# erwincoumans/tiny-differentiable-simulator

Hardware: AMD Instinct MI355X
Metric: env-steps/sec (higher is better)
Workload: dtype f64

## Files before the change

tiny-differentiable-simulator_amd/csrc/tds_oct.hip:

```cpp
#include <hip/hip_runtime.h>
#include <stdlib.h>

#include "tds_device_model.h"
#include "tds_kernels.h"
#include "tds_lanes.h"
#include "tds_step_shared.h"

#ifdef TDS_OCT_PROF
#ifndef TDS_OCT_PROF_WG
#define TDS_OCT_PROF_WG 3
#endif
__device__ unsigned long long tds_oct_prof_buf[32];
__device__ unsigned long long tds_oct_prof_clk[64];
__device__ unsigned long long tds_oct_prof_wg[3 * 2048];
__device__ int tds_oct_prof_iter = 500;
#define OCT_STAMP(k, pin)                                                                       \
  do {                                                                                          \
    unsigned long long t_;                                                                      \
    auto p_ = (pin);        \
    asm volatile("s_memtime %0\n\ts_waitcnt lgkmcnt(0)" : "=s"(t_), "+v"(p_)::"memory");        \
    if (prof_on) prof_t[k] = t_;                                                                \
  } while (0)
#else
#define OCT_STAMP(k, pin) do { } while (0)
#endif

#ifdef TDS_OCT_MARKS
#define OCT_MARK(name) asm volatile("; OCTMARK " name ::: "memory")
#else
#define OCT_MARK(name) do { } while (0)
#endif

namespace {

#define OCT_SYNC()                                             \
  do {                                                         \
    __builtin_amdgcn_fence(__ATOMIC_ACQ_REL, "wavefront");     \
    __builtin_amdgcn_wave_barrier();                           \
  } while (0)

template <int CTRL>
__device__ __forceinline__ double oct_dpp(double v) {
  const int l = __double2loint(v), h = __double2hiint(v);
  const int lo = __builtin_amdgcn_update_dpp(0, l, CTRL, 0xF, 0xF, true);
  const int hi = __builtin_amdgcn_update_dpp(0, h, CTRL, 0xF, 0xF, true);
  return __hiloint2double(hi, lo);
}
template <int CTRL>
__device__ __forceinline__ float oct_dpp(float v) {
  return __int_as_float(__builtin_amdgcn_update_dpp(0, __float_as_int(v), CTRL, 0xF, 0xF, true));
}
template <typename T>
__device__ __forceinline__ T pair_other(T v) { return oct_dpp<0xB1>(v); }
template <int K, typename T>
__device__ __forceinline__ T pair_bcast(T v) { return oct_dpp<(K == 0 ? 0xA0 : 0xF5)>(v); }
template <typename T>
__device__ __forceinline__ T oct_sum(T v) {
  asm volatile("" : "+v"(v));
  v += oct_dpp<0xB1>(v);
  v += oct_dpp<0x4E>(v);
  v += oct_dpp<0x141>(v);
  return v;
}
template <int K>
__device__ __forceinline__ double oct_bcast(double v) {
  const double t = __builtin_amdgcn_update_dpp(0.0, v, 0x150 + K, 0xF, 0x3, false);
  return __builtin_amdgcn_update_dpp(t, v, 0x150 + 8 + K, 0xF, 0xC, false);
}
template <int K>
__device__ __forceinline__ float oct_bcast(float v) {
  const int b = __float_as_int(v);
  const int t = __builtin_amdgcn_update_dpp(0, b, 0x150 + K, 0xF, 0x3, false);
  return __int_as_float(__builtin_amdgcn_update_dpp(t, b, 0x150 + 8 + K, 0xF, 0xC, false));
}

struct OctOff {
  int lcw, legf, swl, qdp, fac, win, xs, cp, stride;
};
struct OctLds {
  static constexpr int LCW = 6;
  static constexpr int ZW = 14;
  static constexpr int Z_B = 10, Z_A = 11, Z_G = 12, Z_HL = 13;
  static constexpr int NCP = 17;
};
__host__ __device__ inline OctOff oct_layout(int in_dim) {
  OctOff o;
  int at = in_dim + 4;
  at = (at + 1) & ~1;
  o.lcw = at;  at += 8 * OctLds::LCW;
  o.legf = at; at += 4 * 3;
  o.swl = at;  at += 8 * 6;
  o.qdp = at;  at += 8;
  o.fac = at;  at += 28;
  o.win = at;  at += 2 * 8 * OctLds::ZW;
  o.xs = at;   at += 3 * OctLds::NCP + 1;
  o.cp = at;   at += 5 * OctLds::NCP + 1;
  at = (at + 1) & ~1;
  while ((((at * 2) & 63) % 8) != 0 || ((at * 2) & 63) == 0 || ((at * 2) & 63) == 32) at += 2;
  o.stride = at;
  return o;
}

struct OctKernArgs {
  const void *mdl, *x_in;
  void *y_out;
  const void *actions;
  void *x_feedback, *obs_out;
  TdsStepCtl ctl;
  int n_envs;
  OctOff O;
};
using TB = TdsOctTab;

#ifdef TDS_OCT_NT
#define OCT_ST(v, p) __builtin_nontemporal_store((v), (p))
#else
#define OCT_ST(v, p) (*(p) = (v))
#endif
#define OCT_BAR()                                                                        \
  do {                                                                                   \
    if constexpr (W2) asm volatile("s_waitcnt lgkmcnt(0)\n\ts_barrier" ::: "memory");    \
    else OCT_SYNC();                                                                     \
  } while (0)

template <typename T, typename TR, bool LOOP, int BUILD>
__device__ __forceinline__ void oct_body(const DevModel<T> *__restrict__ mdl_arg, const TR *x_in, TR *__restrict__ y_out,
                                         const TR *__restrict__ actions, TR *x_feedback ,
                                         TR *__restrict__ obs_out, const TdsStepCtl &ctl_arg, int n_envs, const OctOff &O) {
  extern __shared__ __align__(16) unsigned char tds_oct_smem[];
  T *const sm = reinterpret_cast<T *>(tds_oct_smem);
#ifdef TDS_OCT_PROF
  if (threadIdx.x == 0 && blockIdx.x < 2048) {
    unsigned long long c_;
    asm volatile("s_memrealtime %0\n\ts_waitcnt lgkmcnt(0)" : "=s"(c_)::"memory");
    tds_oct_prof_wg[3 * blockIdx.x] = c_;
  }
#endif
  constexpr bool W2 = BUILD >= 2;
  constexpr int nq = 14, nd = 14, adim = 8, in_dim = nq + nd + adim + 3, w_obs = nq + nd + 2;
  constexpr int NT = W2 ? 128 : 64;
  T *const CT = sm + 8 * O.stride;
  {
    const int t = threadIdx.x;
// ... 66 lines not shown
    asm volatile("s_memtime %0\n\ts_memrealtime %1\n\ts_waitcnt lgkmcnt(0)" : "=s"(c0_), "=s"(c1_)::"memory");
    tds_oct_prof_clk[2 * it] = c0_;
    tds_oct_prof_clk[2 * it + 1] = c1_;
  }
#endif
  const int lane = tid & 7;
  const int grp = (tid & 63) >> 3;
  const int env = blockIdx.x * 8 + grp;
  const bool valid = env < n_envs;
  T *const E = sm + grp * O.stride;
  T *const xr = E;
  const int leg = lane >> 1, pos = lane & 1;
  const int dq = 6 + lane;
  const T *const CL = CT + lane * TB::LSTR;
  typename TdsCtlRef<LOOP>::type ctl = TdsCtlRef<LOOP>::get(ctl_arg, ka_seg + __builtin_offsetof(OctKernArgs, ctl));
  const T dt = CT[TB::SC + TB::DT];
  const int pgs_iters = (int)CT[TB::SC + TB::PGS_ITERATIONS];
  const bool last = it == nsteps - 1;
  OCT_STAMP(0, tid);

  T q, qd, tau;
  T Sl[6], R[9], p[3], sw[6], v[6], a0[6];
  T R5[9], P[3], A4[3], A5[3], pA3[3], pA4[3], pA5[3], v5[6], a5[6];
  T Lc[6], l10, id0, id1, sq0, sq1, my_id, my_sq, Ls[15], ids[6], sq_ids[6], qd_new, qdr_new[6];
  T Cb, Cr[6], It[10];
  T u = T(0), urm = T(0);
  T u_init = T(0), urm_init = T(0);
  int na = 0, NA = 0;

  auto root_frame = [&](T sx, T cx, T sy, T cy, T sz, T cz) {
    R5[0] = cy * cz;                 R5[1] = -cy * sz;                R5[2] = sy;
    R5[3] = sx * sy * cz + cx * sz;  R5[4] = cx * cz - sx * sy * sz;  R5[5] = -sx * cy;
    R5[6] = sx * sz - cx * sy * cz;  R5[7] = cx * sy * sz + sx * cz;  R5[8] = cx * cy;
    P[0] = xr[0] + CT[TB::SC + TB::BASE_T];
    P[1] = xr[1] + CT[TB::SC + TB::BASE_T + 1];
    P[2] = xr[2] + CT[TB::SC + TB::BASE_T + 2];
    A4[0] = T(0); A4[1] = cx; A4[2] = sx;
    A5[0] = sy; A5[1] = -sx * cy; A5[2] = cx * cy;
    pA3[0] = T(0); pA3[1] = P[2]; pA3[2] = -P[1];
    cross3(P, A4, pA4);
    cross3(P, A5, pA5);
  };
  auto times_inertia = [&](const T *I, const T *s, T *F) {
    T t3[3];
    sym3_mulv(I, s, F);
    cross3(I + 6, s + 3, t3);
    F[0] += t3[0];
    F[1] += t3[1];
    F[2] += t3[2];
    cross3(I + 6, s, t3);
    F[3] = I[9] * s[3] - t3[0];
    F[4] = I[9] * s[4] - t3[1];
    F[5] = I[9] * s[5] - t3[2];
  };
  auto dot6 = [&](const T *a, const T *b) -> T { return dot3(a, b) + dot3(a + 3, b + 3); };

  auto main_kin = [&]() {
    OCT_MARK("main_top");
    q = xr[dq];
    qd = xr[nq + dq];
    tau = T(0);
    {
      const int act_i = act_slot;
      if (act_i >= 0) {
        const int var = nq + nd + adim;
        const T kp = xr[var], kd = xr[var + 1], max_force = xr[var + 2];
        const T act_lim = CT[TB::SC + TB::ACTION_LIMIT];
        T a = xr[nq + nd + act_i];
        a = a < act_lim ? a : act_lim;
        a = a > -act_lim ? a : -act_lim;
        const T q_des = CL[TB::IPOSE] + a;
        T f = kp * (q_des - q) + kd * (T(0) - qd);
        f = f > -max_force ? f : -max_force;
        f = f < max_force ? f : max_force;
        tau = f;
      }
      tau -= CL[TB::STIFF] * q + CL[TB::DAMP] * qd;
      asm volatile("" : "+v"(tau));
    }
    OCT_MARK("main_jcalc");
#pragma unroll
    for (int k = 0; k < 6; ++k) Sl[k] = CL[TB::S + k];
    T Rp[9], tp[3];
    {
      T sn, cs;
      tds_sincos(q * CL[TB::ROTF], &sn, &cs);
      const T c1 = T(1) - cs;
      const T nx = CL[TB::NAX], ny = CL[TB::NAX + 1], nz = CL[TB::NAX + 2];
      T RJ[9];
      RJ[0] = cs + c1 * CL[TB::NN + 0];
      RJ[1] = c1 * CL[TB::NN + 1] - sn * nz;
      RJ[2] = c1 * CL[TB::NN + 2] + sn * ny;
      RJ[3] = c1 * CL[TB::NN + 1] + sn * nz;
      RJ[4] = cs + c1 * CL[TB::NN + 3];
      RJ[5] = c1 * CL[TB::NN + 4] - sn * nx;
      RJ[6] = c1 * CL[TB::NN + 2] - sn * ny;
      RJ[7] = c1 * CL[TB::NN + 4] + sn * nx;
      RJ[8] = cs + c1 * CL[TB::NN + 5];
      const T tJ[3] = {Sl[3] * q, Sl[4] * q, Sl[5] * q};
      if (CT[TB::SC + TB::XT_IDENT] != T(0)) {
#pragma unroll
        for (int k = 0; k < 9; ++k) Rp[k] = RJ[k];
#pragma unroll
        for (int k = 0; k < 3; ++k) tp[k] = CL[TB::XT + 9 + k] + tJ[k];
      } else {
        T RT[9], r[3];
#pragma unroll
        for (int k = 0; k < 9; ++k) RT[k] = CL[TB::XT + k];
        mat3_mul(RT, RJ, Rp);
        mat3_mulv(RT, tJ, r);
#pragma unroll
        for (int k = 0; k < 3; ++k) tp[k] = CL[TB::XT + 9 + k] + r[k];
      }
    }
    OCT_MARK("main_rootsincos");
    {
      T rs, rc;
      tds_sincos(xr[3 + (lane < 3 ? lane : 0)], &rs, &rc);
      const T sx = oct_bcast<0>(rs), cx = oct_bcast<0>(rc);
      const T sy = oct_bcast<1>(rs), cy = oct_bcast<1>(rc);
      const T sz = oct_bcast<2>(rs), cz = oct_bcast<2>(rc);
      if constexpr (W2) {
        if (lane < 3) {
          T *const sc = E + O.win + 8 * OctLds::ZW + 96;
          sc[2 * lane] = rs;
          sc[2 * lane + 1] = rc;
        }
      }
      root_frame(sx, cx, sy, cy, sz, cz);
    }
    OCT_MARK("main_rootvel");
    {
      const T d0 = xr[nq + 0], d1 = xr[nq + 1], d2 = xr[nq + 2], d3 = xr[nq + 3], d4 = xr[nq + 4], d5 = xr[nq + 5];
      const T U[3] = {d0, d1, d2};
      const T J3[3] = {d3, T(0), T(0)}, J4[3] = {A4[0] * d4, A4[1] * d4, A4[2] * d4}, J5[3] = {A5[0] * d5, A5[1] * d5, A5[2] * d5};
      const T W4[3] = {J3[0] + J4[0], J3[1] + J4[1], J3[2] + J4[2]};
      const T W5[3] = {W4[0] + J5[0], W4[1] + J5[1], W4[2] + J5[2]};
      T pJ3[3], pJ4[3], pJ5[3];
      cross3(P, J3, pJ3);
      cross3(P, J4, pJ4);
      cross3(P, J5, pJ5);
      const T pW4[3] = {pJ3[0] + pJ4[0], pJ3[1] + pJ4[1], pJ3[2] + pJ4[2]};
      const T pW5[3] = {pW4[0] + pJ5[0], pW4[1] + pJ5[1], pW4[2] + pJ5[2]};
      const T V3[3] = {U[0] + pJ3[0], U[1] + pJ3[1], U[2] + pJ3[2]};
      const T V4[3] = {U[0] + pW4[0], U[1] + pW4[1], U[2] + pW4[2]};
      const T V5[3] = {U[0] + pW5[0], U[1] + pW5[1], U[2] + pW5[2]};
      T a45[3], a55[3], t1[3], t2[3], l3[3], l4[3], l5[3];
      cross3(J3, J4, a45);
      cross3(W4, J5, a55);
      cross3(J3, pJ3, t1);
      cross3(V3, J3, t2);
      l3[0] = t1[0] + t2[0]; l3[1] = t1[1] + t2[1]; l3[2] = t1[2] + t2[2];
      cross3(W4, pJ4, t1);
      cross3(V4, J4, t2);
      l4[0] = t1[0] + t2[0]; l4[1] = t1[1] + t2[1]; l4[2] = t1[2] + t2[2];
      cross3(W5, pJ5, t1);
      cross3(V5, J5, t2);
      l5[0] = t1[0] + t2[0]; l5[1] = t1[1] + t2[1]; l5[2] = t1[2] + t2[2];
#pragma unroll
      for (int k = 0; k < 3; ++k) {
        v5[k] = W5[k];
        v5[3 + k] = V5[k];
        a5[k] = a45[k] + a55[k];
        a5[3 + k] = (l3[k] + l4[k] + l5[k]) - CT[TB::SC + TB::GRAV + k];
      }
    }
    OCT_MARK("main_legs");
    {
      const bool take = pos == 1;
      T Rq[9], pq[3];
#pragma unroll
      for (int k = 0; k < 9; ++k) {
        const T sh = pair_bcast<0>(Rp[k]);
        Rq[k] = take ? sh : ((k == 0 || k == 4 || k == 8) ? T(1) : T(0));
      }
#pragma unroll
      for (int k = 0; k < 3; ++k) {
        const T sh = pair_bcast<0>(tp[k]);
        pq[k] = take ? sh : T(0);
      }
      T Rl[9], pl[3], r[3];
      mat3_mul(Rq, Rp, Rl);
      mat3_mulv(Rq, tp, r);
#pragma unroll
      for (int k = 0; k < 3; ++k) pl[k] = pq[k] + r[k];
      mat3_mul(R5, Rl, R);
      mat3_mulv(R5, pl, r);
      p[0] = P[0] + r[0];
      p[1] = P[1] + r[1];
      p[2] = P[2] + r[2];
      mat3_mulv(R, Sl, sw);
      mat3_mulv(R, Sl + 3, sw + 3);
      T c[3];
      cross3(p, sw, c);
      sw[3] += c[0];
      sw[4] += c[1];
      sw[5] += c[2];
      T vJ[6];
#pragma unroll
      for (int k = 0; k < 6; ++k) vJ[k] = sw[k] * qd;
#pragma unroll
// ... 336 lines not shown
      times_inertia(It, ax3, F3);
      times_inertia(It, ax4, F4);
      times_inertia(It, ax5, F5);
      Sm[0] = m;
      Sm[1] = T(0); Sm[2] = m;
      Sm[3] = T(0); Sm[4] = T(0); Sm[5] = m;
      Sm[6] = F3[3]; Sm[7] = F3[4]; Sm[8] = F3[5]; Sm[9] = dot6(ax3, F3);
      Sm[10] = F4[3]; Sm[11] = F4[4]; Sm[12] = F4[5]; Sm[13] = dot6(ax4, F3); Sm[14] = dot6(ax4, F4);
      Sm[15] = F5[3]; Sm[16] = F5[4]; Sm[17] = F5[5]; Sm[18] = dot6(ax5, F3); Sm[19] = dot6(ax5, F4); Sm[20] = dot6(ax5, F5);
    }
    OCT_SYNC();
    OCT_MARK("main_ldl6");
    {
      const T *const Ssum = E + O.fac;
#pragma unroll
      for (int e = 0; e < 21; ++e) Sm[e] -= Ssum[e];
      static_for<0, 6>([&](auto kc) {
        constexpr int k = decltype(kc)::value;
        const T rs = rsqrt_full<T>(Sm[(k * (k + 1)) / 2 + k]);
        const T inv = rs * rs;
        sq_ids[k] = rs;
        ids[k] = inv;
        T col[6];
        static_for<k + 1, 6>([&](auto rc) {
          constexpr int r = decltype(rc)::value;
          col[r] = Sm[(r * (r + 1)) / 2 + k];
          Ls[(r * (r - 1)) / 2 + k] = col[r] * inv;
        });
        static_for<k + 1, 6>([&](auto rc) {
          constexpr int r = decltype(rc)::value;
          static_for<k + 1, r + 1>([&](auto cc) {
            constexpr int c = decltype(cc)::value;
            Sm[(r * (r + 1)) / 2 + c] -= Ls[(r * (r - 1)) / 2 + k] * col[c];
          });
        });
      });
    }
    OCT_STAMP(4, Ls[14]);
    OCT_MARK("main_fd");
    if constexpr (W2) {
      T *const fac = E + O.fac;
      OCT_SYNC();
      if (lane == 0) {
#pragma unroll
        for (int k = 0; k < 15; ++k) fac[k] = Ls[k];
#pragma unroll
        for (int k = 0; k < 6; ++k) fac[15 + k] = sq_ids[k];
      }
    }
    OCT_MARK("main_dyn_end");
  };
  auto main_fd = [&]() {
    OCT_MARK("main_fd");
    T y = tau - Cb;
    y -= (pos == 1 ? l10 : T(0)) * pair_bcast<0>(y);
    T yr[6];
#pragma unroll
    for (int r = 0; r < 6; ++r) yr[r] = -Cr[r] - oct_sum(Lc[r] * y);
    static_for<1, 6>([&](auto rc) {
      constexpr int r = decltype(rc)::value;
      static_for<0, r>([&](auto cc) {
        constexpr int c = decltype(cc)::value;
        yr[r] -= Ls[(r * (r - 1)) / 2 + c] * yr[c];
      });
    });
    u = -dt * (y * my_sq);
    T sel = yr[0] * sq_ids[0];
#pragma unroll
    for (int r = 1; r < 6; ++r) sel = lane == r ? yr[r] * sq_ids[r] : sel;
    urm = lane < 6 ? -dt * sel : T(0);
    u_init = u;
    urm_init = urm;
    OCT_STAMP(5, u);
  };
  auto main_get_count = [&]() { NA = __builtin_amdgcn_readfirstlane((int)sm[in_dim + 3]); };
  auto help_get_factors = [&]() {
    const T *const fac = E + O.fac;
#pragma unroll
    for (int k = 0; k < 15; ++k) Ls[k] = fac[k];
#pragma unroll
    for (int k = 0; k < 6; ++k) sq_ids[k] = fac[15 + k];
  };

  auto rows_geom = [&](int wi) {
      OCT_MARK("rows_geom");
      const int nr = 3 * NA, nwin = (nr + 7) >> 3;
      const int w0 = (wi % nwin) * 8;
      T *const row = E + O.win + (wi & 1) * (8 * OctLds::ZW) + lane * OctLds::ZW;
      const T *const cpx = E + O.cp;
      const T *const swl = E + O.swl;
      const int s = w0 + lane;
      const int tk = (s >= NA ? 1 : 0) + (s >= 2 * NA ? 1 : 0);
      const int a = s - tk * NA;
      const bool real = s < nr && a < na;
      const int ac = real ? a : 0;
      const T Pc[3] = {cpx[0 * OctLds::NCP + ac], cpx[1 * OctLds::NCP + ac], cpx[2 * OctLds::NCP + ac]};
      const T dist = cpx[3 * OctLds::NCP + ac];
      const T owner = cpx[4 * OctLds::NCP + ac];
      const T *const dir = CT + TB::SC + TB::NB + 3 * tk;
      const T e[3] = {dir[0], dir[1], dir[2]};
      const int ol = real ? (int)owner : 8;
      const bool on_leg = ol < 8;
      const int hl = on_leg ? (ol & ~1) : 0;
      const bool ank = on_leg && (ol & 1);
      T sh[6], sa[6];
#pragma unroll
      for (int c = 0; c < 6; ++c) {
        sh[c] = swl[hl * 6 + c];
        sa[c] = swl[(hl + 1) * 6 + c];
      }
      const T qh = xr[nq + 6 + hl], qa = xr[nq + 6 + hl + 1];
      T mo[3];
      cross3(Pc, e, mo);
      const T j0 = dot3(e, sh + 3) + dot3(mo, sh), j1 = dot3(e, sa + 3) + dot3(mo, sa);
      const T z0 = on_leg ? j0 : T(0), z1 = ank ? j1 : T(0);
      T zr[6];
      zr[0] = e[0];
      zr[1] = e[1];
      zr[2] = e[2];
      zr[3] = dot3(e, pA3) + mo[0];
      zr[4] = dot3(e, pA4) + dot3(mo, A4);
      zr[5] = dot3(e, pA5) + dot3(mo, A5);
      const T vrow = ((z0 * qh + z1 * qa) + (zr[0] * xr[nq + 0] + zr[1] * xr[nq + 1])) +
                     ((zr[2] * xr[nq + 2] + zr[3] * xr[nq + 3]) + (zr[4] * xr[nq + 4] + zr[5] * xr[nq + 5]));
      const T crow = tk == 0 ? (T(1) + CT[TB::SC + TB::RESTITUTION]) * vrow - CT[TB::SC + TB::ERP_OVER_DT] * dist : vrow;
      row[0] = z0;
      row[1] = z1;
#pragma unroll
      for (int rr = 0; rr < 6; ++rr) row[2 + rr] = real ? zr[rr] : T(0);
      row[8] = T(0);
      row[9] = T(0);
      row[OctLds::Z_B] = real ? crow : T(0);
      row[OctLds::Z_A] = real ? T(1) : T(0);
      row[OctLds::Z_HL] = on_leg ? (T)hl : T(-2);
      OCT_MARK("rows_geom_end");
  };
  auto rows_leg = [&](int wi) {
      OCT_MARK("rows_leg");
      T *const row = E + O.win + (wi & 1) * (8 * OctLds::ZW) + lane * OctLds::ZW;
      const T *const lcw = E + O.lcw;
      T z0 = row[0], z1 = row[1], zr[6];
#pragma unroll
      for (int rr = 0; rr < 6; ++rr) zr[rr] = row[2 + rr];
      const T hlv = row[OctLds::Z_HL];
      const int hl = hlv >= T(0) ? (int)hlv : 0;
      T lch[6], lca[6];
#pragma unroll
      for (int c = 0; c < 6; ++c) {
        lch[c] = lcw[hl * OctLds::LCW + c];
        lca[c] = lcw[(hl + 1) * OctLds::LCW + c];
      }
      const T *const lf = E + O.legf + (hl >> 1) * 3;
      const T lf0 = lf[0], lf1 = lf[1], lf2 = lf[2];
      z1 -= lf0 * z0;
#pragma unroll
      for (int rr = 0; rr < 6; ++rr) row[2 + rr] = zr[rr] - (lch[rr] * z0 + lca[rr] * z1);
      row[0] = z0 * lf1;
      row[1] = z1 * lf2;
  };
  auto rows_root = [&](int wi) {
      OCT_MARK("rows_root");
      T *const row = E + O.win + (wi & 1) * (8 * OctLds::ZW) + lane * OctLds::ZW;
      const T z0 = row[0], z1 = row[1];
      T zr[6];
#pragma unroll
      for (int rr = 0; rr < 6; ++rr) zr[rr] = row[2 + rr];
      const bool real = row[OctLds::Z_A] != T(0);
      static_for<1, 6>([&](auto rc) {
        constexpr int rr = decltype(rc)::value;
        static_for<0, rr>([&](auto cc) {
          constexpr int c = decltype(cc)::value;
          zr[rr] -= Ls[(rr * (rr - 1)) / 2 + c] * zr[c];
        });
      });
#pragma unroll
      for (int rr = 0; rr < 6; ++rr) zr[rr] *= sq_ids[rr];
      const T g = ((z0 * z0 + z1 * z1) + (zr[0] * zr[0] + zr[1] * zr[1])) + ((zr[2] * zr[2] + zr[3] * zr[3]) + (zr[4] * zr[4] + zr[5] * zr[5]));
      const T ai = real ? rcp_full<T>(g + CT[TB::SC + TB::CFM]) : T(0);
#pragma unroll
      for (int rr = 0; rr < 6; ++rr) row[2 + rr] = zr[rr];
      row[OctLds::Z_A] = ai;
      row[OctLds::Z_G] = g;
      OCT_MARK("rows_root_end");
      OCT_STAMP(10, ai);
  };
  auto main_sweep = [&](int wi) {
      OCT_MARK("sweep");
      const int nr = 3 * NA, nwin = (nr + 7) >> 3;
      const int pit = wi / nwin;
      const int w0 = (wi - pit * nwin) * 8;
      const T *const Zs = E + O.win + (wi & 1) * (8 * OctLds::ZW);
      T *const xs = E + O.xs;
      const T my_hip = (T)(lane & ~1);
      const T mu = CT[TB::SC + TB::FRICTION], rest = CT[TB::SC + TB::RESTITUTION];
      const int wn = nr - w0 < 8 ? nr - w0 : 8;
      const int k_n = NA - w0 < 0 ? 0 : (NA - w0 < wn ? NA - w0 : wn);
      struct Ops { T zs, zm, b, a, g, hl, sd, xo; };
      auto request = [&](int k, Ops &o, auto firstc, auto normalc) {
        constexpr bool FIRST = decltype(firstc)::value, NORMAL = decltype(normalc)::value;
        const T *const row = Zs + k * OctLds::ZW;
        o.zs = row[pos];
        o.zm = row[2 + lane];
        o.b = row[OctLds::Z_B];
        o.a = row[OctLds::Z_A];
        o.hl = row[OctLds::Z_HL];
        if constexpr (!FIRST) {
          o.g = row[OctLds::Z_G];
          o.xo = xs[w0 + k];
        }
        if constexpr (!NORMAL) o.sd = xs[w0 + k - ((w0 + k >= 2 * NA) ? 2 : 1) * NA];
      };
      auto process = [&](int k, const Ops &o, auto firstc, auto normalc) {
        constexpr bool FIRST = decltype(firstc)::value, NORMAL = decltype(normalc)::value;
        const T zl = o.hl == my_hip ? o.zs : T(0);
        T jw;
        if constexpr (NORMAL) jw = oct_sum(zl * (u + rest * u_init) + o.zm * (urm + rest * urm_init));
        else jw = oct_sum(zl * u + o.zm * urm);
        T xn;
        if constexpr (FIRST) xn = (o.b - jw) * o.a;
        else xn = (o.b - (jw - o.g * o.xo)) * o.a;
        if constexpr (NORMAL) {
          xn = max_t<T>(xn, T(0));
          xn = min_t<T>(xn, T(100000));
        } else {
          const T hi = mu * max_t<T>(o.sd, T(0));
          xn = max_t<T>(xn, -hi);
          xn = min_t<T>(xn, hi);
        }
        T dx;
        if constexpr (FIRST) dx = xn;
        else dx = xn - o.xo;
        u += zl * dx;
        urm += o.zm * dx;
        xs[w0 + k] = xn;
      };
      auto run = [&](int k0, int k1, auto firstc, auto normalc) {
        if (k0 >= k1) return;
        Ops A, B;
        request(k0, A, firstc, normalc);
        for (int k = k0; k < k1; k += 2) {
          request(k + 1 < k1 ? k + 1 : k, B, firstc, normalc);
          process(k, A, firstc, normalc);
          if (k + 1 < k1) {
            request(k + 2 < k1 ? k + 2 : k + 1, A, firstc, normalc);
            process(k + 1, B, firstc, normalc);
          }
        }
      };
      if (pit == 0) {
        run(0, k_n, std::true_type{}, std::true_type{});
        run(k_n, wn, std::true_type{}, std::false_type{});
      } else {
        run(0, k_n, std::false_type{}, std::true_type{});
        run(k_n, wn, std::false_type{}, std::false_type{});
      }
      OCT_SYNC();
      OCT_MARK("sweep_end");
  };
  auto windows = [&]() -> int { return NA > 0 ? pgs_iters * ((3 * NA + 7) >> 3) : 0; };

  bool done_reg = false, done_in_reg = false;
  auto main_fin = [&]() {
    OCT_MARK("main_fin");
    OCT_STAMP(6, u);
    {
      T w = u * my_sq;
      T wr[6];
      static_for<0, 6>([&](auto rc) {
        constexpr int r = decltype(rc)::value;
        wr[r] = oct_bcast<r>(urm) * sq_ids[r];
      });
      static_for<0, 5>([&](auto ic) {
        constexpr int r = 4 - decltype(ic)::value;
        static_for<r + 1, 6>([&](auto cc) {
          constexpr int c = decltype(cc)::value;
          wr[r] -= Ls[(c * (c - 1)) / 2 + r] * wr[c];
        });
      });
#pragma unroll
      for (int r = 0; r < 6; ++r) w -= Lc[r] * wr[r];
      w -= (pos == 0 ? l10 : T(0)) * pair_bcast<1>(w);
      qd_new = qd - w;
#pragma unroll
      for (int r = 0; r < 6; ++r) qdr_new[r] = xr[nq + r] - wr[r];
    }
    OCT_MARK("main_integrate");
    T qn0, qn2, qo0;
    const int rm = (int)CT[TB::SC + TB::REWARD_MODE];
    const T inv_dt = CT[TB::SC + TB::INV_DT];
    OCT_SYNC();
    {
      T qn_root[6];
#pragma unroll
      for (int r = 0; r < 6; ++r) qn_root[r] = xr[r] + qdr_new[r] * dt;
      const T q_old0 = xr[0];
      qn0 = qn_root[0];
      qn2 = qn_root[2];
      qo0 = q_old0;
      OCT_SYNC();
      if (lane == 0) {
#pragma unroll
        for (int r = 0; r < 6; ++r) {
          xr[r] = qn_root[r];
          xr[nq + r] = qdr_new[r];
        }
      }
      xr[dq] = q + qd_new * dt;
      xr[nq + dq] = qd_new;
      if (lane == 0) {
        xr[in_dim] = q_old0;
        xr[in_dim + 3] = T(0);
      }
    }
    OCT_SYNC();
    OCT_MARK("main_reward");
    done_in_reg = rm == TDS_REWARD_ANT;
    if (rm == TDS_REWARD_ANT) {
      const T vel_x = (qn0 - qo0) * inv_dt;
      done_reg = qn2 < T(0.26);
      const T reward = done_reg ? T(0) : vel_x;
      if (lane == 0) {
        xr[in_dim + 1] = done_reg ? T(1) : T(0);
        xr[in_dim + 2] = reward;
      }
    } else {
      T rs = T(0), rc = T(1);
      if (rm == TDS_REWARD_LAIKAGO) sincos_t<T>(lane < 3 ? xr[3 + lane] * T(0.5) : T(0), &rs, &rc);
      const T s1 = oct_bcast<1>(rs), c1 = oct_bcast<1>(rc), s2 = oct_bcast<2>(rs), c2 = oct_bcast<2>(rc);
      if (lane == 0) {
        bool done = false;
        T reward = T(0);
        if (rm == TDS_REWARD_LAIKAGO) {
          const T sp = rs, cp = rc, st = s1, ct = c1, ss = s2, cs2 = c2;
          const T qx = sp * ct * cs2 - cp * st * ss;
          const T qy = cp * st * cs2 + sp * ct * ss;
          const T qz = cp * ct * ss - sp * st * cs2;
          const T qw = cp * ct * cs2 + sp * st * ss;
          const T sq = T(2) / (qx * qx + qy * qy + qz * qz + qw * qw);
// ... 98 lines not shown
                  hi = (unsigned)__double2hiint(dv);
                }
              }
            }
            const unsigned long long bits = ((unsigned long long)hi << 32) | (unsigned long long)lo;
            const size_t unit_at = row0 / per_unit + (size_t)uu;
            if (on) __hip_atomic_store(tds_global((unsigned long long *)ctl.obs_ring) + unit_at, bits, __ATOMIC_RELAXED, __HIP_MEMORY_SCOPE_AGENT);
            const bool to_peers = on && (!rd_only || tail);
            for (int p0 = 0; p0 < np; p0 += 4) {
              const unsigned long long *const b0 = tds_global(tab[p0]), *const b1 = tds_global(tab[p0 + 1]), *const b2 = tds_global(tab[p0 + 2]),
                                       *const b3 = tds_global(tab[p0 + 3]);
              const size_t po = (size_t)ctl.peer_off / 8 + unit_at;
              if (to_peers) {
                using G64 = __attribute__((address_space(1))) unsigned long long;
                __hip_atomic_store((G64 *)((unsigned long long *)b0 + po), bits, __ATOMIC_RELAXED, __HIP_MEMORY_SCOPE_SYSTEM);
                if (p0 + 1 < np) __hip_atomic_store((G64 *)((unsigned long long *)b1 + po), bits, __ATOMIC_RELAXED, __HIP_MEMORY_SCOPE_SYSTEM);
                if (p0 + 2 < np) __hip_atomic_store((G64 *)((unsigned long long *)b2 + po), bits, __ATOMIC_RELAXED, __HIP_MEMORY_SCOPE_SYSTEM);
                if (p0 + 3 < np) __hip_atomic_store((G64 *)((unsigned long long *)b3 + po), bits, __ATOMIC_RELAXED, __HIP_MEMORY_SCOPE_SYSTEM);
              }
            }
          }
        } else if (valid) {
          const size_t at = ((size_t)slot * ctl.obs_envs + env) * w_obs;
          constexpr int NB = (w_obs + 7) / 8;
          T ov[NB];
#pragma unroll
          for (int k = 0; k < NB; ++k) {
            const int i = lane + 8 * k;
            const T rv = xr[i >= w_obs ? 0 : (i < nq + nd ? i : (i == nq + nd ? in_dim + 2 : in_dim + 1))];
            ov[k] = i < 2 ? T(0) : rv;
          }
#pragma unroll
          for (int k = 0; k < NB; ++k) {
            const int i = lane + 8 * k;
            if (i >= w_obs) continue;
            const T vv = ov[k];
            if (rf & TDS_RING_OBS_F32) {
              float *const pp = tds_global((float *)ctl.obs_ring) + at + i;
              if (rf & TDS_RING_NOFENCE) __hip_atomic_store(pp, (float)vv, __ATOMIC_RELAXED, __HIP_MEMORY_SCOPE_AGENT);
              else OCT_ST((float)vv, pp);
            } else {
              TR *const pp = tds_global((TR *)ctl.obs_ring) + at + i;
              if (rf & TDS_RING_NOFENCE) __hip_atomic_store(pp, (TR)vv, __ATOMIC_RELAXED, __HIP_MEMORY_SCOPE_AGENT);
              else OCT_ST((TR)vv, pp);
            }
            if (np > 0 && (i >= nq + nd || !rd_only)) {
              for (int pr = 0; pr < np; ++pr) {
                char *const pb = (char *)tds_global(((void *const __attribute__((address_space(4))) *)(const __attribute__((address_space(4))) void *)ctl.peer_ring)[pr]) + ctl.peer_off;
                if (rf & TDS_RING_OBS_F32) __hip_atomic_store((float *)pb + (at + i), (float)vv, __ATOMIC_RELAXED, __HIP_MEMORY_SCOPE_SYSTEM);
                else __hip_atomic_store((TR *)pb + (at + i), (TR)vv, __ATOMIC_RELAXED, __HIP_MEMORY_SCOPE_SYSTEM);
              }
            }
          }
        }
        if (last && ctl.peer_arrive != nullptr) tds_signal_slot(ctl, slot);
      }
    }
    if (valid && last) {
      for (int i = lane; i < nq + nd; i += 8) {
        const TR vv = (TR)xr[i];
        if (obs_out != nullptr) obs_out[(size_t)env * w_obs + i] = i < 2 ? TR(0) : vv;
        if (x_feedback != nullptr) x_feedback[(size_t)env * in_dim + i] = vv;
      }
      if (lane == 0 && obs_out != nullptr) {
        obs_out[(size_t)env * w_obs + nq + nd] = (TR)xr[in_dim + 2];
        obs_out[(size_t)env * w_obs + nq + nd + 1] = (TR)xr[in_dim + 1];
      }
    }
    OCT_MARK("help_rec_end");
    OCT_STAMP(11, tid);
  };

  if constexpr (W2) {
    if (wv == 0) {
      main_kin();
      OCT_BAR();
      main_dyn();
      OCT_BAR();
      main_dyn2();
      OCT_BAR();
      main_get_count();
      main_fd();
      const int nw = windows();
      for (int wi = 0; wi < nw; ++wi) {
        OCT_BAR();
        if (wi == 0) OCT_STAMP(12, tid);
        main_sweep(wi);
        if (wi == 0) OCT_STAMP(13, u);
      }
      main_fin();
      main_pool();
      OCT_BAR();
    } else {
      OCT_BAR();
      help_np();
      if (NA > 0) rows_geom(0);
      OCT_BAR();
      if (NA > 0) rows_leg(0);
      help_poses();
      OCT_BAR();
      const int nw = windows();
      if (nw > 0) {
        if constexpr (TDS_OCT_PRIO == 2) __builtin_amdgcn_s_setprio(3);
        help_get_factors();
        rows_root(0);
        if constexpr (TDS_OCT_PRIO == 2) __builtin_amdgcn_s_setprio(0);
      }
      for (int wi = 0; wi < nw; ++wi) {
        if (wi > 0) {
          rows_geom(wi);
          rows_leg(wi);
          rows_root(wi);
        }
        OCT_BAR();
      }
      OCT_BAR();
      help_rec();
    }
  } else {
    main_kin();
    OCT_SYNC();
    help_np();
    help_poses();
    main_dyn();
    OCT_SYNC();
    main_dyn2();
    main_fd();
    const int nw = windows();
    for (int wi = 0; wi < nw; ++wi) {
      rows_geom(wi);
      rows_leg(wi);
      rows_root(wi);
      OCT_SYNC();
      main_sweep(wi);
    }
    main_fin();
    main_pool();
    OCT_SYNC();
    help_rec();
    if constexpr (LOOP) OCT_SYNC();
  }
#ifdef TDS_OCT_PROF
  if (prof_on && (tid & 63) == 0) {
#pragma unroll
    for (int k = 16; k < 24; ++k)
      if (is_main) tds_oct_prof_buf[k] = prof_t[k];
#pragma unroll
    for (int k = 0; k < 14; ++k)
      if (((k < 8 || k >= 12) && is_main) || (k >= 8 && k < 12 && is_help)) tds_oct_prof_buf[k] = prof_t[k];
    if (is_help) tds_oct_prof_buf[15] = (unsigned long long)NA;
  }
#endif
  if constexpr (LOOP) {
    act_blk = act_blk + 1 >= ctl_arg.act_blocks ? 0 : act_blk + 1;
    y_slot = y_slot + 1 >= ctl_arg.y_slots ? 0 : y_slot + 1;
    o_slot = o_slot + 1 >= ctl_arg.obs_slots ? 0 : o_slot + 1;
  }
  }
#ifdef TDS_OCT_PROF
  if (threadIdx.x == 0 && blockIdx.x < 2048) {
    unsigned long long c_;
    asm volatile("s_waitcnt vmcnt(0)\n\ts_memrealtime %0\n\ts_waitcnt lgkmcnt(0)" : "=s"(c_)::"memory");
    tds_oct_prof_wg[3 * blockIdx.x + 2] = c_;
  }
#endif
}

template <typename T, typename TR, bool LOOP, int BUILD>
__global__ __launch_bounds__(BUILD >= 2 ? 128 : 64) __attribute__((amdgpu_waves_per_eu(BUILD == 2 ? 2 : 1, BUILD == 2 ? 2 : 1)))
void tds_oct_kernel(const DevModel<T> *__restrict__ mdl_arg, const TR *x_in, TR *__restrict__ y_out,
                    const TR *__restrict__ actions, TR *x_feedback, TR *__restrict__ obs_out, TdsStepCtl ctl_arg, int n_envs,
                    OctOff O) {
  oct_body<T, TR, LOOP, BUILD>(mdl_arg, x_in, y_out, actions, x_feedback, obs_out, ctl_arg, n_envs, O);
}
template <typename T, typename TR, bool LOOP>
__global__ __launch_bounds__(128) __attribute__((amdgpu_waves_per_eu(2, 2), amdgpu_num_vgpr(120)))
void tds_oct_kernel_beside(const DevModel<T> *__restrict__ mdl_arg, const TR *x_in, TR *__restrict__ y_out,
                           const TR *__restrict__ actions, TR *x_feedback, TR *__restrict__ obs_out, TdsStepCtl ctl_arg,
                           int n_envs, OctOff O) {
  oct_body<T, TR, LOOP, 4>(mdl_arg, x_in, y_out, actions, x_feedback, obs_out, ctl_arg, n_envs, O);
}

}

#ifdef TDS_OCT_PROF
extern "C" int tds_oct_prof_workgroups(unsigned long long *out, int n_wg) {
  return hipMemcpyFromSymbol(out, HIP_SYMBOL(tds_oct_prof_wg), (size_t)3 * n_wg * sizeof(unsigned long long)) == hipSuccess ? 0 : -1;
}
extern "C" int tds_oct_prof_clocks(unsigned long long *out64) {
  return hipMemcpyFromSymbol(out64, HIP_SYMBOL(tds_oct_prof_clk), 64 * sizeof(unsigned long long)) == hipSuccess ? 0 : -1;
}
extern "C" int tds_oct_prof_read(unsigned long long *out32, int iter) {
  if (out32 && hipMemcpyFromSymbol(out32, HIP_SYMBOL(tds_oct_prof_buf), 32 * sizeof(unsigned long long)) != hipSuccess) return -1;
  if (iter >= 0 && hipMemcpyToSymbol(HIP_SYMBOL(tds_oct_prof_iter), &iter, sizeof(int)) != hipSuccess) return -1;
  return 0;
}
#endif

int tds_oct_lds_bytes(int input_dim) { return oct_layout(input_dim).stride * (int)sizeof(double); }
int tds_oct_workgroup_bytes(int input_dim) {
  return (oct_layout(input_dim).stride * 8 + TdsOctTab::TOTAL) * (int)sizeof(double);
}

template <typename T, typename TR>
int tds_launch_oct(const DevModel<T> *d_model, const DevModel<T> &h_model, const TR *x_in, TR *y_out, const TR *actions,
                   TR *x_feedback, TR *obs_out, int n_envs, hipStream_t stream, const TdsStepCtl &ctl, int build) {
  const OctOff O = oct_layout(h_model.input_dim);
  const int blocks = (n_envs + 7) / 8;
  const size_t shmem = ((size_t)O.stride * 8 + TdsOctTab::TOTAL) * sizeof(T);
  const bool one_step = ctl.nsub == 1 && ctl.obs_ring == nullptr && ctl.y_ring == nullptr;
#define OCT_LAUNCH(LOOP_, B_)                                                                                                 \
  hipLaunchKernelGGL((tds_oct_kernel<T, TR, LOOP_, B_>), dim3(blocks), dim3(B_ >= 2 ? 128 : 64), shmem, stream, d_model, x_in, \
                     y_out, actions, x_feedback, obs_out, ctl, n_envs, O)
  if (build == 4) {
    if (one_step)
      hipLaunchKernelGGL((tds_oct_kernel_beside<T, TR, false>), dim3(blocks), dim3(128), shmem, stream, d_model, x_in, y_out, actions,
                         x_feedback, obs_out, ctl, n_envs, O);
// ... 20 lines not shown
```

tiny-differentiable-simulator_amd/csrc/tds_step_shared.h:

```cpp
#pragma once
#include <hip/hip_runtime.h>

#include "tds_kernels.h"

#define TDS_AS4 __attribute__((address_space(4)))

template <typename P>
__device__ __forceinline__ P *tds_global(P *p) {
#if defined(__HIP_DEVICE_COMPILE__)
  __builtin_assume(!__builtin_amdgcn_is_shared((const void *)p) && !__builtin_amdgcn_is_private((const void *)p));
#endif
  return p;
}

template <bool LOOP, typename S>
struct TdsKaRef {
  using type = const S &;
  static __device__ __forceinline__ type get(const S &param, const TDS_AS4 char *) { return param; }
};
template <typename S>
struct TdsKaRef<true, S> {
  using type = const TDS_AS4 S &;
  static __device__ __forceinline__ type get(const S &, const TDS_AS4 char *at) { return *(const TDS_AS4 S *)at; }
};
template <bool LOOP>
using TdsCtlRef = TdsKaRef<LOOP, TdsStepCtl>;

static __device__ __forceinline__ void tds_sincos(double x, double *sn, double *cs) {
  const bool big = !(__builtin_fabs(x) < 1.0e5);
  const double k = __builtin_rint(x * 6.36619772367581382433e-01);
  double r = __builtin_fma(-k, 1.57079632679489655800e+00, x);
  r = __builtin_fma(-k, 6.12323399573676603587e-17, r);
  const int q = (int)k;
  const double z = r * r;
  double ps = __builtin_fma(z, 1.58969099521155010221e-10, -2.50507602534068634195e-08);
  ps = __builtin_fma(z, ps, 2.75573137070700676789e-06);
  ps = __builtin_fma(z, ps, -1.98412698298579493134e-04);
  ps = __builtin_fma(z, ps, 8.33333333332248946124e-03);
  ps = __builtin_fma(z, ps, -1.66666666666666324348e-01);
  const double s0 = __builtin_fma(z * r, ps, r);
  double pc = __builtin_fma(z, -1.13596475577881948265e-11, 2.08757232129817482790e-09);
  pc = __builtin_fma(z, pc, -2.75573143513906633035e-07);
  pc = __builtin_fma(z, pc, 2.48015872894767294178e-05);
  pc = __builtin_fma(z, pc, -1.38888888888741095749e-03);
  pc = __builtin_fma(z, pc, 4.16666666666666019037e-02);
  const double c0 = __builtin_fma(z * z, pc, __builtin_fma(z, -0.5, 1.0));
  const bool swap = (q & 1) != 0;
  const double ss = swap ? c0 : s0, cc = swap ? s0 : c0;
  double s_ = (q & 2) ? -ss : ss, c_ = ((q + 1) & 2) ? -cc : cc;
  if (__builtin_expect(__any(big), 0)) {
    double s2, c2;
    sincos(x, &s2, &c2);
    s_ = big ? s2 : s_;
    c_ = big ? c2 : c_;
  }
  *sn = s_;
  *cs = c_;
}
static __device__ __forceinline__ void tds_sincos(float x, float *sn, float *cs) { sincosf(x, sn, cs); }

template <typename CTL>
__device__ __forceinline__ unsigned tds_peer_count_in(const CTL &ctl, int pslot) {
  __builtin_amdgcn_s_waitcnt(0x0f70);
  if ((ctl.ring_flags & TDS_RING_PEER_RELEASE) != 0) __builtin_amdgcn_fence(__ATOMIC_RELEASE, "");
  unsigned tok = 0u;
  if ((threadIdx.x & 63) == 0) {
    constexpr unsigned SUB = TDS_PEER_SUB;
    const unsigned g = gridDim.x, j = blockIdx.x % SUB;
    const unsigned n1 = (g - j + SUB - 1u) / SUB;
    unsigned *const base = tds_global(ctl.peer_arrive) + (size_t)pslot * TDS_PEER_ARRIVE_STRIDE;
    tok = atomicInc(base + j * TDS_PEER_LINE, n1 - 1u);
  }
  return tok;
}
template <typename CTL>
__device__ __forceinline__ void tds_peer_finish(const CTL &ctl, int pslot, unsigned tok) {
  if ((threadIdx.x & 63) == 0) {
    constexpr unsigned SUB = TDS_PEER_SUB;
    const unsigned g = gridDim.x, j = blockIdx.x % SUB;
    const unsigned n1 = (g - j + SUB - 1u) / SUB;
    const unsigned n2 = g < SUB ? g : SUB;
    unsigned *const base = tds_global(ctl.peer_arrive) + (size_t)pslot * TDS_PEER_ARRIVE_STRIDE;
    if (tok == n1 - 1u) {
      if (atomicInc(base + 32 * TDS_PEER_LINE, n2 - 1u) == n2 - 1u) {
        const size_t fi = (size_t)ctl.peer_flag_off + (size_t)pslot * (size_t)ctl.peer_flag_stride;
        if ((ctl.ring_flags & TDS_RING_PEER_RELEASE) != 0) __builtin_amdgcn_fence(__ATOMIC_ACQ_REL, "");
        for (int pr = 0; pr <= ctl.n_peers; ++pr)
          __hip_atomic_store(ctl.peer_flags[pr] + fi, ctl.peer_epoch, __ATOMIC_RELAXED, __HIP_MEMORY_SCOPE_SYSTEM);
      }
    }
  }
}
template <typename CTL>
__device__ __forceinline__ void tds_signal_slot(const CTL &ctl, int pslot) {
  if (ctl.peer_arrive != nullptr) {
    tds_peer_finish(ctl, pslot, tds_peer_count_in(ctl, pslot));
  } else if (ctl.progress != nullptr) {
    if (ctl.ring_flags & TDS_RING_NOFENCE)
      __builtin_amdgcn_s_waitcnt(0x0f70);
    else
      __builtin_amdgcn_fence(__ATOMIC_RELEASE, "agent");
    if ((threadIdx.x & 63) == 0)
      __hip_atomic_fetch_add(tds_global(ctl.progress) + pslot, 1ull, __ATOMIC_RELAXED, __HIP_MEMORY_SCOPE_AGENT);
  }
}

static __device__ __forceinline__ bool tds_obs_travels(int ring_flags, bool reward_or_done) {
  return reward_or_done || (ring_flags & TDS_RING_PEER_REWARD_DONE) == 0;
}

template <int EPW, int W, typename TR, typename CTL, typename COL>
__device__ __forceinline__ void tds_obs_store_wide(const CTL &ctl, int slot, int wl, int w_rt, COL col) {
  using T = decltype(col(0, 0));
  const int w = W > 0 ? W : w_rt;
  const int rf = ctl.ring_flags;
  const size_t row0 = ((size_t)slot * ctl.obs_envs + (size_t)blockIdx.x * EPW) * (size_t)w;
  const bool f32w = (rf & TDS_RING_OBS_F32) != 0 || sizeof(TR) == 4;
  const int per_unit = f32w ? 2 : 1;
  const int n_units = (EPW * w) / per_unit;
  const int np = ctl.n_peers;
  const unsigned long long *const TDS_AS4 *tab = (const unsigned long long *const TDS_AS4 *)(const TDS_AS4 void *)ctl.peer_ring;
  for (int u0 = 0; u0 < n_units; u0 += 64) {
    const int u = u0 + wl;
    const bool on = u < n_units;
    unsigned lo = 0u, hi = 0u;
    bool tail = false;
#pragma unroll
    for (int c = 0; c < 2; ++c) {
      if (c < per_unit) {
        const int f = on ? u * per_unit + c : 0;
        int e = 0;
        if constexpr (W > 0) {
          e = f / W;
        } else {
#pragma unroll
          for (int k = 1; k < EPW; ++k) e += f >= k * w ? 1 : 0;
        }
        const int i = f - e * w;
        const T v = i < 2 ? T(0) : col(e, i);
        tail = tail || i >= w - 2;
        if (f32w) {
          const unsigned b = (unsigned)__float_as_int((float)v);
// ... 54 lines not shown
```

Before: 587.4 million.

## Software-pipeline contact sweep rows into DPP reductions and pair sincos evaluations

Rewrites the per-window contact sweep as a fully unrolled compile-time row sequence. Each row's LDS loads for the next row are split into three parts and placed between the DPP steps of the octet reduction, using scheduling barriers to hide LDS latency behind the cross-lane dependency chain. Window offsets and the first-iteration flag are now tracked incrementally by the caller instead of computed with divisions. The joint-angle and root-angle sincos are also evaluated together in an interleaved two-lane polynomial to expose ILP. The price is larger code size and register pressure from the unrolled rows, plus rigid sched_barrier ordering.

```diff
diff --git a/tiny-differentiable-simulator_amd/csrc/tds_oct.hip b/tiny-differentiable-simulator_amd/csrc/tds_oct.hip
--- a/tiny-differentiable-simulator_amd/csrc/tds_oct.hip
+++ b/tiny-differentiable-simulator_amd/csrc/tds_oct.hip
@@ -27,8 +27,10 @@
 
 #ifdef TDS_OCT_MARKS
 #define OCT_MARK(name) asm volatile("; OCTMARK " name ::: "memory")
+#define OCT_ROWMARK(name) asm volatile("; OCTROW " name)
 #else
 #define OCT_MARK(name) do { } while (0)
+#define OCT_ROWMARK(name) do { } while (0)
 #endif
 
 namespace {
@@ -59,6 +61,23 @@
   asm volatile("" : "+v"(v));
   v += oct_dpp<0xB1>(v);
   v += oct_dpp<0x4E>(v);
+  v += oct_dpp<0x141>(v);
+  return v;
+}
+template <typename T, typename F0, typename F1, typename F2>
+__device__ __forceinline__ T oct_sum_filled(T v, F0 f0, F1 f1, F2 f2) {
+  asm volatile("" : "+v"(v));
+  __builtin_amdgcn_sched_barrier(0);
+  f0();
+  __builtin_amdgcn_sched_barrier(0);
+  v += oct_dpp<0xB1>(v);
+  __builtin_amdgcn_sched_barrier(0);
+  f1();
+  __builtin_amdgcn_sched_barrier(0);
+  v += oct_dpp<0x4E>(v);
+  __builtin_amdgcn_sched_barrier(0);
+  f2();
+  __builtin_amdgcn_sched_barrier(0);
   v += oct_dpp<0x141>(v);
   return v;
 }
@@ -291,9 +310,10 @@
 #pragma unroll
     for (int k = 0; k < 6; ++k) Sl[k] = CL[TB::S + k];
     T Rp[9], tp[3];
+    T rs, rc;
     {
       T sn, cs;
-      tds_sincos(q * CL[TB::ROTF], &sn, &cs);
+      tds_sincos2(q * CL[TB::ROTF], xr[3 + (lane < 3 ? lane : 0)], &sn, &cs, &rs, &rc);
       const T c1 = T(1) - cs;
       const T nx = CL[TB::NAX], ny = CL[TB::NAX + 1], nz = CL[TB::NAX + 2];
       T RJ[9];
@@ -324,8 +344,6 @@
     }
     OCT_MARK("main_rootsincos");
     {
-      T rs, rc;
-      tds_sincos(xr[3 + (lane < 3 ? lane : 0)], &rs, &rc);
       const T sx = oct_bcast<0>(rs), cx = oct_bcast<0>(rc);
       const T sy = oct_bcast<1>(rs), cy = oct_bcast<1>(rc);
       const T sz = oct_bcast<2>(rs), cz = oct_bcast<2>(rc);
@@ -828,10 +846,9 @@
     for (int k = 0; k < 6; ++k) sq_ids[k] = fac[15 + k];
   };
 
-  auto rows_geom = [&](int wi) {
+  auto rows_geom = [&](int wi, int w0) {
       OCT_MARK("rows_geom");
-      const int nr = 3 * NA, nwin = (nr + 7) >> 3;
-      const int w0 = (wi % nwin) * 8;
+      const int nr = 3 * NA;
       T *const row = E + O.win + (wi & 1) * (8 * OctLds::ZW) + lane * OctLds::ZW;
       const T *const cpx = E + O.cp;
       const T *const swl = E + O.swl;
@@ -930,44 +947,52 @@
       OCT_MARK("rows_root_end");
       OCT_STAMP(10, ai);
   };
-  auto main_sweep = [&](int wi) {
+  auto main_sweep = [&](int wi, int w0, bool first_it) {
       OCT_MARK("sweep");
-      const int nr = 3 * NA, nwin = (nr + 7) >> 3;
-      const int pit = wi / nwin;
-      const int w0 = (wi - pit * nwin) * 8;
+      const int nr = 3 * NA;
       const T *const Zs = E + O.win + (wi & 1) * (8 * OctLds::ZW);
-      T *const xs = E + O.xs;
+      T *const xw = E + O.xs + w0;
       const T my_hip = (T)(lane & ~1);
       const T mu = CT[TB::SC + TB::FRICTION], rest = CT[TB::SC + TB::RESTITUTION];
       const int wn = nr - w0 < 8 ? nr - w0 : 8;
       const int k_n = NA - w0 < 0 ? 0 : (NA - w0 < wn ? NA - w0 : wn);
+      const int k2 = 2 * NA - w0;
+      const T *const sd1 = xw - NA, *const sd2 = sd1 - NA;
+      T cap = T(100000);
+      asm volatile("" : "+s"(cap));
       struct Ops { T zs, zm, b, a, g, hl, sd, xo; };
-      auto request = [&](int k, Ops &o, auto firstc, auto normalc) {
+      auto request = [&](auto partc, auto kc, Ops &o, auto firstc, auto fromnormalc) {
+        constexpr int part = decltype(partc)::value, k = decltype(kc)::value;
+        constexpr bool FIRST = decltype(firstc)::value, FROM_NORMAL = decltype(fromnormalc)::value;
+        const T *const row = Zs + k * OctLds::ZW;
+        if constexpr (part == 0) {
+          o.zs = row[pos];
+          o.zm = row[2 + lane];
+        } else if constexpr (part == 1) {
+          o.hl = row[OctLds::Z_HL];
+          if constexpr (!FIRST) o.g = row[OctLds::Z_G];
+          o.b = row[OctLds::Z_B];
+          o.a = row[OctLds::Z_A];
+        } else {
+          if constexpr (FROM_NORMAL) o.sd = sd1[k];
+          else o.sd = (k >= k2 ? sd2 : sd1)[k];
+          if constexpr (!FIRST) o.xo = xw[k];
+        }
+      };
+      auto process = [&](auto kc, const Ops &o, auto firstc, auto normalc, auto f0, auto f1, auto f2) {
+        constexpr int k = decltype(kc)::value;
         constexpr bool FIRST = decltype(firstc)::value, NORMAL = decltype(normalc)::value;
-        const T *const row = Zs + k * OctLds::ZW;
-        o.zs = row[pos];
-        o.zm = row[2 + lane];
-        o.b = row[OctLds::Z_B];
-        o.a = row[OctLds::Z_A];
-        o.hl = row[OctLds::Z_HL];
-        if constexpr (!FIRST) {
-          o.g = row[OctLds::Z_G];
-          o.xo = xs[w0 + k];
-        }
-        if constexpr (!NORMAL) o.sd = xs[w0 + k - ((w0 + k >= 2 * NA) ? 2 : 1) * NA];
-      };
-      auto process = [&](int k, const Ops &o, auto firstc, auto normalc) {
-        constexpr bool FIRST = decltype(firstc)::value, NORMAL = decltype(normalc)::value;
+        asm volatile("" : : "v"(o.zs), "v"(o.zm), "v"(o.hl));
         const T zl = o.hl == my_hip ? o.zs : T(0);
         T jw;
-        if constexpr (NORMAL) jw = oct_sum(zl * (u + rest * u_init) + o.zm * (urm + rest * urm_init));
-        else jw = oct_sum(zl * u + o.zm * urm);
+        if constexpr (NORMAL) jw = oct_sum_filled(zl * (u + rest * u_init) + o.zm * (urm + rest * urm_init), f0, f1, f2);
+        else jw = oct_sum_filled(zl * u + o.zm * urm, f0, f1, f2);
         T xn;
         if constexpr (FIRST) xn = (o.b - jw) * o.a;
         else xn = (o.b - (jw - o.g * o.xo)) * o.a;
         if constexpr (NORMAL) {
           xn = max_t<T>(xn, T(0));
-          xn = min_t<T>(xn, T(100000));
+          xn = min_t<T>(xn, cap);
         } else {
           const T hi = mu * max_t<T>(o.sd, T(0));
           xn = max_t<T>(xn, -hi);
@@ -978,28 +1003,49 @@
         else dx = xn - o.xo;
         u += zl * dx;
         urm += o.zm * dx;
-        xs[w0 + k] = xn;
+        xw[k] = xn;
       };
-      auto run = [&](int k0, int k1, auto firstc, auto normalc) {
-        if (k0 >= k1) return;
-        Ops A, B;
-        request(k0, A, firstc, normalc);
-        for (int k = k0; k < k1; k += 2) {
-          request(k + 1 < k1 ? k + 1 : k, B, firstc, normalc);
-          process(k, A, firstc, normalc);
-          if (k + 1 < k1) {
-            request(k + 2 < k1 ? k + 2 : k + 1, A, firstc, normalc);
-            process(k + 1, B, firstc, normalc);
-          }
+      auto window = [&](auto firstc) {
+        Ops ops[2];
+        using I0 = std::integral_constant<int, 0>;
+        using I1 = std::integral_constant<int, 1>;
+        using I2 = std::integral_constant<int, 2>;
+        request(I0{}, I0{}, ops[0], firstc, std::false_type{});
+        request(I1{}, I0{}, ops[0], firstc, std::false_type{});
+        request(I2{}, I0{}, ops[0], firstc, std::false_type{});
+#define OCT_ROW(K, NORMALC)                                                                    \
+        {                                                                                      \
+          using KC = std::integral_constant<int, K>;                                           \
+          using KN = std::integral_constant<int, (K) + 1>;                                     \
+          auto next = [&](auto partc) {                                                        \
+            if constexpr ((K) < 7) request(partc, KN{}, ops[((K) + 1) & 1], firstc, NORMALC{}); \
+          };                                                                                   \
+          if constexpr (decltype(firstc)::value) {                                             \
+            if constexpr (NORMALC::value) OCT_ROWMARK("first_normal");                         \
+            else OCT_ROWMARK("first_friction");                                                \
+          } else {                                                                             \
+            if constexpr (NORMALC::value) OCT_ROWMARK("later_normal");                         \
+            else OCT_ROWMARK("later_friction");                                                \
+          }                                                                                    \
+          process(KC{}, ops[(K) & 1], firstc, NORMALC{}, [&]() { next(I0{}); }, [&]() { next(I1{}); }, \
+                  [&]() { next(I2{}); });                                                      \
         }
+#define OCT_ROW_N(K) if (k_n <= (K)) break; OCT_ROW(K, std::true_type)
+#define OCT_ROW_F(K) case K: if (wn <= (K)) break; OCT_ROW(K, std::false_type)
+        do {
+          OCT_ROW_N(0) OCT_ROW_N(1) OCT_ROW_N(2) OCT_ROW_N(3) OCT_ROW_N(4) OCT_ROW_N(5) OCT_ROW_N(6) OCT_ROW_N(7)
+        } while (0);
+        if (NA == 1) ops[1].sd = xw[0];
+        switch (k_n) {
+          OCT_ROW_F(0) OCT_ROW_F(1) OCT_ROW_F(2) OCT_ROW_F(3) OCT_ROW_F(4) OCT_ROW_F(5) OCT_ROW_F(6) OCT_ROW_F(7)
+          default: break;
+        }
+#undef OCT_ROW_F
+#undef OCT_ROW_N
+#undef OCT_ROW
       };
-      if (pit == 0) {
-        run(0, k_n, std::true_type{}, std::true_type{});
-        run(k_n, wn, std::true_type{}, std::false_type{});
-      } else {
-        run(0, k_n, std::false_type{}, std::true_type{});
-        run(k_n, wn, std::false_type{}, std::false_type{});
-      }
+      if (first_it) window(std::true_type{});
+      else window(std::false_type{});
       OCT_SYNC();
       OCT_MARK("sweep_end");
   };
@@ -1264,11 +1310,18 @@
       main_get_count();
       main_fd();
       const int nw = windows();
+      int w0 = 0;
+      bool first_it = true;
       for (int wi = 0; wi < nw; ++wi) {
         OCT_BAR();
         if (wi == 0) OCT_STAMP(12, tid);
-        main_sweep(wi);
+        main_sweep(wi, w0, first_it);
         if (wi == 0) OCT_STAMP(13, u);
+        w0 += 8;
+        if (w0 >= 3 * NA) {
+          w0 = 0;
+          first_it = false;
+        }
       }
       main_fin();
       main_pool();
@@ -1276,7 +1329,7 @@
     } else {
       OCT_BAR();
       help_np();
-      if (NA > 0) rows_geom(0);
+      if (NA > 0) rows_geom(0, 0);
       OCT_BAR();
       if (NA > 0) rows_leg(0);
       help_poses();
@@ -1288,13 +1341,15 @@
         rows_root(0);
         if constexpr (TDS_OCT_PRIO == 2) __builtin_amdgcn_s_setprio(0);
       }
+      int w0 = 0;
       for (int wi = 0; wi < nw; ++wi) {
         if (wi > 0) {
-          rows_geom(wi);
+          rows_geom(wi, w0);
           rows_leg(wi);
           rows_root(wi);
         }
         OCT_BAR();
+        w0 = w0 + 8 >= 3 * NA ? 0 : w0 + 8;
       }
       OCT_BAR();
       help_rec();
@@ -1309,12 +1364,19 @@
     main_dyn2();
     main_fd();
     const int nw = windows();
+    int w0 = 0;
+    bool first_it = true;
     for (int wi = 0; wi < nw; ++wi) {
-      rows_geom(wi);
+      rows_geom(wi, w0);
       rows_leg(wi);
       rows_root(wi);
       OCT_SYNC();
-      main_sweep(wi);
+      main_sweep(wi, w0, first_it);
+      w0 += 8;
+      if (w0 >= 3 * NA) {
+        w0 = 0;
+        first_it = false;
+      }
     }
     main_fin();
     main_pool();
diff --git a/tiny-differentiable-simulator_amd/csrc/tds_step_shared.h b/tiny-differentiable-simulator_amd/csrc/tds_step_shared.h
--- a/tiny-differentiable-simulator_amd/csrc/tds_step_shared.h
+++ b/tiny-differentiable-simulator_amd/csrc/tds_step_shared.h
@@ -26,7 +26,7 @@
 template <bool LOOP>
 using TdsCtlRef = TdsKaRef<LOOP, TdsStepCtl>;
 
-static __device__ __forceinline__ void tds_sincos(double x, double *sn, double *cs) {
+static __host__ __device__ __forceinline__ void tds_sincos(double x, double *sn, double *cs) {
   const bool big = !(__builtin_fabs(x) < 1.0e5);
   const double k = __builtin_rint(x * 6.36619772367581382433e-01);
   double r = __builtin_fma(-k, 1.57079632679489655800e+00, x);
@@ -48,7 +48,12 @@
   const bool swap = (q & 1) != 0;
   const double ss = swap ? c0 : s0, cc = swap ? s0 : c0;
   double s_ = (q & 2) ? -ss : ss, c_ = ((q + 1) & 2) ? -cc : cc;
-  if (__builtin_expect(__any(big), 0)) {
+#if defined(__HIP_DEVICE_COMPILE__)
+  const bool any_big = __any(big);
+#else
+  const bool any_big = big;
+#endif
+  if (__builtin_expect(any_big, 0)) {
     double s2, c2;
     sincos(x, &s2, &c2);
     s_ = big ? s2 : s_;
@@ -57,7 +62,71 @@
   *sn = s_;
   *cs = c_;
 }
-static __device__ __forceinline__ void tds_sincos(float x, float *sn, float *cs) { sincosf(x, sn, cs); }
+static __host__ __device__ __forceinline__ void tds_sincos(float x, float *sn, float *cs) { sincosf(x, sn, cs); }
+
+static __host__ __device__ __forceinline__ void tds_sincos2(double x0, double x1, double *sn0, double *cs0, double *sn1, double *cs1) {
+  constexpr double two_over_pi = 6.36619772367581382433e-01, pio2_hi = 1.57079632679489655800e+00, pio2_lo = 6.12323399573676603587e-17;
+  constexpr double S1 = -1.66666666666666324348e-01, S2 = 8.33333333332248946124e-03, S3 = -1.98412698298579493134e-04,
+                   S4 = 2.75573137070700676789e-06, S5 = -2.50507602534068634195e-08, S6 = 1.58969099521155010221e-10;
+  constexpr double C1 = 4.16666666666666019037e-02, C2 = -1.38888888888741095749e-03, C3 = 2.48015872894767294178e-05,
+                   C4 = -2.75573143513906633035e-07, C5 = 2.08757232129817482790e-09, C6 = -1.13596475577881948265e-11;
+  const bool big0 = !(__builtin_fabs(x0) < 1.0e5), big1 = !(__builtin_fabs(x1) < 1.0e5);
+  const double k0 = __builtin_rint(x0 * two_over_pi), k1 = __builtin_rint(x1 * two_over_pi);
+  double r0 = __builtin_fma(-k0, pio2_hi, x0), r1 = __builtin_fma(-k1, pio2_hi, x1);
+  r0 = __builtin_fma(-k0, pio2_lo, r0);
+  r1 = __builtin_fma(-k1, pio2_lo, r1);
+  const int q0 = (int)k0, q1 = (int)k1;
+  const double z0 = r0 * r0, z1 = r1 * r1;
+  double ps0 = __builtin_fma(z0, S6, S5), ps1 = __builtin_fma(z1, S6, S5);
+  ps0 = __builtin_fma(z0, ps0, S4);
+  ps1 = __builtin_fma(z1, ps1, S4);
+  ps0 = __builtin_fma(z0, ps0, S3);
+  ps1 = __builtin_fma(z1, ps1, S3);
+  ps0 = __builtin_fma(z0, ps0, S2);
+  ps1 = __builtin_fma(z1, ps1, S2);
+  ps0 = __builtin_fma(z0, ps0, S1);
+  ps1 = __builtin_fma(z1, ps1, S1);
+  const double s00 = __builtin_fma(z0 * r0, ps0, r0), s01 = __builtin_fma(z1 * r1, ps1, r1);
+  double pc0 = __builtin_fma(z0, C6, C5), pc1 = __builtin_fma(z1, C6, C5);
+  pc0 = __builtin_fma(z0, pc0, C4);
+  pc1 = __builtin_fma(z1, pc1, C4);
+  pc0 = __builtin_fma(z0, pc0, C3);
+  pc1 = __builtin_fma(z1, pc1, C3);
+  pc0 = __builtin_fma(z0, pc0, C2);
+  pc1 = __builtin_fma(z1, pc1, C2);
+  pc0 = __builtin_fma(z0, pc0, C1);
+  pc1 = __builtin_fma(z1, pc1, C1);
+  const double c00 = __builtin_fma(z0 * z0, pc0, __builtin_fma(z0, -0.5, 1.0)), c01 = __builtin_fma(z1 * z1, pc1, __builtin_fma(z1, -0.5, 1.0));
+  const bool swap0 = (q0 & 1) != 0, swap1 = (q1 & 1) != 0;
+  const double ss0 = swap0 ? c00 : s00, cc0 = swap0 ? s00 : c00, ss1 = swap1 ? c01 : s01, cc1 = swap1 ? s01 : c01;
+  double s0_ = (q0 & 2) ? -ss0 : ss0, c0_ = ((q0 + 1) & 2) ? -cc0 : cc0;
+  double s1_ = (q1 & 2) ? -ss1 : ss1, c1_ = ((q1 + 1) & 2) ? -cc1 : cc1;
+#if defined(__HIP_DEVICE_COMPILE__)
+  const bool any0 = __any(big0), any1 = __any(big1);
+#else
+  const bool any0 = big0, any1 = big1;
+#endif
+  if (__builtin_expect(any0, 0)) {
+    double s2, c2;
+    sincos(x0, &s2, &c2);
+    s0_ = big0 ? s2 : s0_;
+    c0_ = big0 ? c2 : c0_;
+  }
+  if (__builtin_expect(any1, 0)) {
+    double s2, c2;
+    sincos(x1, &s2, &c2);
+    s1_ = big1 ? s2 : s1_;
+    c1_ = big1 ? c2 : c1_;
+  }
+  *sn0 = s0_;
+  *cs0 = c0_;
+  *sn1 = s1_;
+  *cs1 = c1_;
+}
+static __host__ __device__ __forceinline__ void tds_sincos2(float x0, float x1, float *sn0, float *cs0, float *sn1, float *cs1) {
+  sincosf(x0, sn0, cs0);
+  sincosf(x1, sn1, cs1);
+}
 
 template <typename CTL>
 __device__ __forceinline__ unsigned tds_peer_count_in(const CTL &ctl, int pslot) {
```

Result: no change. 583.8 million (-0.6%).
